# ejmahler/RustFFT

Measured on NVIDIA H100. Metric: batched complex-FFT GFLOP/s (5N log2 N), f32 forward, N=2^10..2^20, batch=4096/GPU, higher is better.
Workload: dtype f32

## Files before the change

rustfft_b200/csrc/common.h:

```cpp
#pragma once

#include <cstddef>
#include <cstdint>

#if defined(__CUDACC__)
#define B2_HD __host__ __device__ __forceinline__
#define B2_D __device__ __forceinline__
#else
#define B2_HD inline
#define B2_D inline
#endif

#if defined(__CUDA_ARCH__)
#define B2_UNROLL _Pragma("unroll")
#else
#define B2_UNROLL
#endif

#if !defined(B2_TW_ALL)
#if !defined(B2_TW_FEW)
#define B2_TW_FEW 1
#endif
#if !defined(B2_TWROW_FEW)
#define B2_TWROW_FEW 1
#endif
#endif

namespace b2 {

template <typename T>
struct alignas(2 * sizeof(T)) cx {
    T x, y;
};

template <typename T> B2_HD cx<T> mk(T x, T y) { cx<T> r; r.x = x; r.y = y; return r; }

template <typename T> B2_HD cx<T> operator+(cx<T> a, cx<T> b) { return mk<T>(a.x + b.x, a.y + b.y); }
template <typename T> B2_HD cx<T> operator-(cx<T> a, cx<T> b) { return mk<T>(a.x - b.x, a.y - b.y); }
template <typename T> B2_HD cx<T> cmul(cx<T> a, cx<T> w) {
#if defined(__CUDA_ARCH__)
    if constexpr (sizeof(T) == 4) return mk<T>(__fmaf_rn(-a.y, w.y, __fmul_rn(a.x, w.x)), __fmaf_rn(a.x, w.y, __fmul_rn(a.y, w.x)));
#endif
    return mk<T>(a.x * w.x - a.y * w.y, a.x * w.y + a.y * w.x);
}
template <typename T> B2_HD cx<T> cmulc(cx<T> a, cx<T> w) {
#if defined(__CUDA_ARCH__)
    if constexpr (sizeof(T) == 4) return mk<T>(__fmaf_rn(a.y, w.y, __fmul_rn(a.x, w.x)), __fmaf_rn(-a.x, w.y, __fmul_rn(a.y, w.x)));
#endif
    return mk<T>(a.x * w.x + a.y * w.y, a.y * w.x - a.x * w.y);
}
template <typename T> B2_HD cx<T> scale(cx<T> a, T s) { return mk<T>(a.x * s, a.y * s); }
template <typename T> B2_HD cx<T> axpy(cx<T> a, T s, cx<T> b) {
#if defined(__CUDA_ARCH__)
    if constexpr (sizeof(T) == 4) return mk<T>(__fmaf_rn(b.x, s, a.x), __fmaf_rn(b.y, s, a.y));
#endif
    return mk<T>(a.x + s * b.x, a.y + s * b.y);
}
template <typename T> B2_HD cx<T> conj(cx<T> a) { return mk<T>(a.x, -a.y); }
template <typename T> B2_HD cx<T> mul_mi(cx<T> a) { return mk<T>(a.y, -a.x); }
template <typename T> B2_HD cx<T> add_mi(cx<T> a, cx<T> b) { return mk<T>(a.x + b.y, a.y - b.x); }
template <typename T> B2_HD cx<T> sub_mi(cx<T> a, cx<T> b) { return mk<T>(a.x - b.y, a.y + b.x); }
template <typename T> B2_HD cx<T> swap_ri(cx<T> a) { return mk<T>(a.y, a.x); }

template <typename T> B2_HD cx<T> ldg(const cx<T>* p) {
#if defined(__CUDA_ARCH__)
    cx<T> r;
    if constexpr (sizeof(T) == 4) {
        asm("ld.global.nc.L1::evict_last.v2.f32 {%0, %1}, [%2];" : "=f"(r.x), "=f"(r.y) : "l"(p));
    } else {
        asm("ld.global.nc.L1::evict_last.v2.f64 {%0, %1}, [%2];" : "=d"(r.x), "=d"(r.y) : "l"(p));
    }
    return r;
#else
    return *p;
#endif
}
template <typename T> B2_HD cx<T> ldg_stream(const cx<T>* p) {
#if defined(__CUDA_ARCH__)
    cx<T> r;
    if constexpr (sizeof(T) == 4) {
        asm("ld.global.nc.L1::no_allocate.v2.f32 {%0, %1}, [%2];" : "=f"(r.x), "=f"(r.y) : "l"(p));
    } else {
        asm("ld.global.nc.L1::no_allocate.v2.f64 {%0, %1}, [%2];" : "=d"(r.x), "=d"(r.y) : "l"(p));
    }
    return r;
#else
    return *p;
#endif
}
B2_HD uint32_t ldg_u32(const uint32_t* p) {
#if defined(__CUDA_ARCH__)
    return __ldg(p);
#else
    return *p;
#endif
}

#if defined(__CUDACC__)
B2_D unsigned long long l2_evict_first() {
    unsigned long long p;
    asm("createpolicy.fractional.L2::evict_first.b64 %0, 1.0;" : "=l"(p));
    return p;
}
B2_D unsigned long long l2_evict_last() {
    unsigned long long p;
    asm("createpolicy.fractional.L2::evict_last.b64 %0, 1.0;" : "=l"(p));
    return p;
}
#endif
template <typename T> B2_HD cx<T> ld_stream(const cx<T>* p) {
#if defined(__CUDA_ARCH__)
    cx<T> r;
    if constexpr (sizeof(T) == 4) {
        asm volatile("ld.global.L1::no_allocate.L2::cache_hint.v2.f32 {%0, %1}, [%2], %3;"
                     : "=f"(r.x), "=f"(r.y) : "l"(p), "l"(l2_evict_first()));
    } else {
        asm volatile("ld.global.L1::no_allocate.L2::cache_hint.v2.f64 {%0, %1}, [%2], %3;"
                     : "=d"(r.x), "=d"(r.y) : "l"(p), "l"(l2_evict_first()));
    }
    return r;
#else
    return *p;
#endif
}
template <typename T> B2_HD void st_stream(cx<T>* p, cx<T> v) {
#if defined(__CUDA_ARCH__)
    if constexpr (sizeof(T) == 4) {
        asm volatile("st.global.L1::no_allocate.L2::cache_hint.v2.f32 [%0], {%1, %2}, %3;" ::"l"(p), "f"(v.x), "f"(v.y),
                     "l"(l2_evict_first()) : "memory");
    } else {
        asm volatile("st.global.L1::no_allocate.L2::cache_hint.v2.f64 [%0], {%1, %2}, %3;" ::"l"(p), "d"(v.x), "d"(v.y),
                     "l"(l2_evict_first()) : "memory");
    }
#else
    *p = v;
#endif
}
template <typename T> B2_HD cx<T> ld_cs(const cx<T>* p) {
#if defined(__CUDA_ARCH__)
    if constexpr (sizeof(T) == 4) {
        float2 v = __ldcs(reinterpret_cast<const float2*>(p));
        return mk<T>(v.x, v.y);
    } else {
        double2 v = __ldcs(reinterpret_cast<const double2*>(p));
        return mk<T>(v.x, v.y);
    }
#else
    return *p;
#endif
}
template <typename T> B2_HD void st_cs(cx<T>* p, cx<T> v) {
#if defined(__CUDA_ARCH__)
    if constexpr (sizeof(T) == 4) {
        __stcs(reinterpret_cast<float2*>(p), make_float2(v.x, v.y));
    } else {
        __stcs(reinterpret_cast<double2*>(p), make_double2(v.x, v.y));
    }
// ... 77 lines not shown
```

rustfft_b200/csrc/engine.h:

```cpp
#pragma once
#include "butterfly.h"
#include "common.h"

namespace b2 {

B2_HD constexpr int hibit(int r) {
    int h = 1;
    while (2 * h <= r) h *= 2;
    return h;
}

B2_HD constexpr int ilog2_c(int r) {
    int l = 0;
    while ((1 << (l + 1)) <= r) ++l;
    return l;
}

enum Map { JF = 0, FF = 1 };

template <typename T_, int L_, int E_, int F_, typename RL_, int PS_ = 4>
struct Geo {
    using T = T_;
    using RL = RL_;
    static constexpr int L = L_, E = E_, F = F_, PS = PS_;
    static constexpr int TP = L / E;
    static constexpr int NT = F * TP;
    static constexpr int NS = RL::N;
    static constexpr int LPAD = L + (PS ? (L >> PS) : 0);
    static constexpr int UNIT = 128 / (2 * (int)sizeof(T_));
    static constexpr int LPR = (LPAD + UNIT - 1) / UNIT * UNIT;
    static constexpr int LP = (F <= 1) ? LPAD : (F >= UNIT ? LPR + 1 : LPR + UNIT / F);
    static constexpr int SMEM_ELEMS = (NS > 1) ? F * LP : 0;
    static constexpr int TW_ELEMS = RL::tw_total();
    static constexpr bool POW2 = RL::all_pow2() && ((TP & (TP - 1)) == 0);
    static B2_HD int sidx(int f, int e) { return f * LP + e + (PS ? (e >> PS) : 0); }
    static_assert(RL::product() == L, "radices must multiply to L");
    static_assert(L % E == 0, "E must divide L");
};

template <class G, Map M>
B2_HD void tid_to_fj(int tid, int& f, int& j) {
    if (M == JF) {
        f = tid / G::TP;
        j = tid - f * G::TP;
    } else {
        j = tid / G::F;
        f = tid - j * G::F;
    }
}

template <class G, Map M0, Map M1>
struct Engine {
    using T = typename G::T;
    using RL = typename G::RL;
    static constexpr int E = G::E;

    template <int S>
    struct TwRegs {
        static constexpr int R = RL::get(S);
        static constexpr int Q = E / R;
        static constexpr int LG = ilog2_c(R);
        cx<T> w[Q][LG > 0 ? LG : 1];
    };
    template <int S>
    static B2_HD void load_tw(int j, const cx<T>* tw, TwRegs<S>& t) {
        constexpr int R = RL::get(S);
        constexpr int p = RL::product(S);
        constexpr int Q = E / R;
        B2_UNROLL
        for (int u = 0; u < Q; ++u) {
            const int i = j + u * G::TP;
            const int k = (p == 1) ? 0 : (i % p);
            const cx<T>* tp = tw + RL::tw_offset(S) + k;
            B2_UNROLL
            for (int l = 0; l < TwRegs<S>::LG; ++l) t.w[u][l] = ldg(tp + ((1 << l) - 1) * p);
        }
    }

    template <int S>
    static B2_HD void stage(int f, int j, cx<T> (&v)[E], cx<T>* smem, const cx<T>* tw, const TwRegs<S>* pre = nullptr) {
        constexpr int R = RL::get(S);
        constexpr int p = RL::product(S);
        constexpr int Q = E / R;
        constexpr bool last = (S == G::NS - 1);
        static_assert(E % R == 0, "every radix must divide E");
        cx<T> out[E];
        B2_UNROLL
        for (int u = 0; u < Q; ++u) {
            const int i = j + u * G::TP;
            const int k = (p == 1) ? 0 : (i % p);
            cx<T> a[R];
            B2_UNROLL
            for (int r = 0; r < R; ++r) a[r] = v[u + r * Q];
            if (S > 0) {
                const cx<T>* t = tw + RL::tw_offset(S) + k;
#if defined(B2_TW_FEW)
                if constexpr (R >= 8 && (R & (R - 1)) == 0 && sizeof(T) == 4) {
                    cx<T> w[R];
                    B2_UNROLL
                    for (int r = 1, l = 0; r < R; r <<= 1, ++l) w[r] = pre ? pre->w[u][l] : ldg(t + (r - 1) * p);
                    B2_UNROLL
                    for (int r = 3; r < R; ++r)
                        if (r & (r - 1)) {
                            const int hi = hibit(r);
                            w[r] = cmul(w[hi], w[r - hi]);
                        }
                    B2_UNROLL
                    for (int r = 1; r < R; ++r) a[r] = cmul(a[r], w[r]);
                } else
#endif
                {
                    B2_UNROLL
                    for (int r = 1; r < R; ++r) a[r] = cmul(a[r], ldg(t + (r - 1) * p));
                }
            }
            Bfly<R, T>::run(a);
            if (last) {
                B2_UNROLL
                for (int m = 0; m < R; ++m) out[u + m * Q] = a[m];
            } else {
                const int base = (i - k) * R + k;
                if constexpr (G::POW2) {
                    cx<T>* wp = smem + G::sidx(f, base);
                    B2_UNROLL
                    for (int m = 0; m < R; ++m) wp[m * p + (G::PS ? ((m * p) >> G::PS) : 0)] = a[m];
                } else {
                    B2_UNROLL
                    for (int m = 0; m < R; ++m) smem[G::sidx(f, base + m * p)] = a[m];
                }
            }
        }
        if (last) {
            B2_UNROLL
            for (int q = 0; q < E; ++q) v[q] = out[q];
        }
    }

    template <int S>
    static B2_HD void read(int f, int j, cx<T> (&v)[E], const cx<T>* smem) {
        if constexpr (G::POW2) {
            const cx<T>* rp = smem + G::sidx(f, j);
            B2_UNROLL
            for (int q = 0; q < E; ++q) v[q] = rp[G::TP * q + (G::PS ? ((G::TP * q) >> G::PS) : 0)];
        } else {
            B2_UNROLL
            for (int q = 0; q < E; ++q) v[q] = smem[G::sidx(f, j + G::TP * q)];
        }
    }

    static constexpr int NPHASE = 2 * G::NS - 1;

    template <int P>
    static B2_HD void owner(int tid, int& f, int& j) {
        if (P == 0)
            tid_to_fj<G, M0>(tid, f, j);
        else
            tid_to_fj<G, M1>(tid, f, j);
    }
    static B2_HD void out_owner(int tid, int& f, int& j) { owner<NPHASE - 1>(tid, f, j); }

    template <int P>
    static B2_HD void phase(int tid, cx<T> (&v)[E], cx<T>* smem, const cx<T>* tw) {
        int f, j;
        owner<P>(tid, f, j);
        if constexpr (P == 0) {
            stage<0>(f, j, v, smem, tw);
        } else if constexpr (P % 2 == 1) {
            read<(P + 1) / 2>(f, j, v, smem);
        } else {
            stage<P / 2>(f, j, v, smem, tw);
        }
    }
    static B2_HD void last_phase_pre(int tid, cx<T> (&v)[E], cx<T>* smem, const cx<T>* tw, const TwRegs<G::NS - 1>& pre) {
        int f, j;
        owner<NPHASE - 1>(tid, f, j);
        stage<G::NS - 1>(f, j, v, smem, tw, &pre);
    }
};

}
```

rustfft_b200/csrc/fused.h:

```cpp
#pragma once
#include "kernels.h"

namespace b2 {

template <class KA, class KB, int NG_, int NS_>
struct FusedKernel {
    using T = typename KA::T;
    static constexpr int NG = NG_;
    static constexpr int NSTAGE = NS_;
    static constexpr int NTG = KA::NT;
    static_assert(KA::NT == KB::NT, "both passes use the same consumer-group size");
    static_assert(KA::TILE_BYTES == KB::TILE_BYTES, "both passes move tiles of the same size");
    static_assert(NTG % 32 == 0 && NSTAGE <= 8 && NG <= 8, "geometry");
    static constexpr int NT = NG * NTG + 96;
    static constexpr int NQ = 2;
    static constexpr size_t STAGE_BYTES = ((KA::SMEM_BYTES > KB::SMEM_BYTES ? KA::SMEM_BYTES : KB::SMEM_BYTES) + 127) / 128 * 128;
    static constexpr size_t CTRL_BYTES = 512;
    static constexpr size_t SMEM_BYTES = (size_t)NSTAGE * STAGE_BYTES + CTRL_BYTES + 128;
    struct Params {
        typename KA::Params a;
        typename KB::Params b;
        FlowSched sched;
        uint32_t* ctl;
        unsigned long long* trace;
        uint32_t flags;
    };
};

static constexpr uint32_t FUSED_TRACE_CTAS = 16, FUSED_TRACE_WORDS = 4096;
inline uint64_t fused_trace_bytes() { return (uint64_t)FUSED_TRACE_CTAS * 4 * FUSED_TRACE_WORDS * 8; }

#if defined(__CUDACC__)
struct FusedTrace {
    unsigned long long* base;
    uint32_t n;
    B2_D void init(unsigned long long* trace, int role) {
        base = (trace != nullptr && blockIdx.x < FUSED_TRACE_CTAS) ? trace + ((size_t)blockIdx.x * 4 + role) * FUSED_TRACE_WORDS : nullptr;
        n = 0;
    }
    B2_D void stamp(uint32_t tag) {
        if (base != nullptr && n + 1 < FUSED_TRACE_WORDS) {
            unsigned long long t;
            asm volatile("mov.u64 %0, %%globaltimer;" : "=l"(t));
            base[n++] = (t << 8) | tag;
        }
    }
    B2_D void finish() {
        if (base != nullptr) base[FUSED_TRACE_WORDS - 1] = n;
    }
};
B2_D void red_release_add1(uint32_t* p) { asm volatile("red.release.gpu.global.add.u32 [%0], 1;" ::"l"(p) : "memory"); }
B2_D uint32_t ld_acquire_u32(const uint32_t* p) {
    uint32_t v;
    asm volatile("ld.acquire.gpu.global.u32 %0, [%1];" : "=r"(v) : "l"(p) : "memory");
    return v;
}
B2_D void fused_spin(uint32_t* ctl, const uint32_t* ctr, uint32_t target) {
    uint32_t spins = 0;
    while (ld_acquire_u32(ctr) < target) {
        __nanosleep(spins < 64 ? 20 : 200);
        if (++spins > (1u << 22) || (spins > 4096 && ld_relaxed_u32(ctl + 1) != 0)) {
            atomicExch(ctl + 1, 1u);
            break;
        }
    }
}

template <class KT, int P>
struct GroupPhases {
    static B2_D void run(const typename KT::Params& p, uint32_t bid, int ltid, typename KT::Regs& r, cx<typename KT::T>* buf, int bar_id,
                         uint64_t* release) {
        KT::template phase<P>(p, bid, ltid, r, buf);
        if constexpr (P + 2 < KT::NPHASE) {
            tma::named_bar_sync(bar_id, KT::NT);
            if constexpr (P + 3 == KT::NPHASE) {
                if (release != nullptr && ltid == 0) tma::mbar_arrive(release);
            }
            GroupPhases<KT, P + 1>::run(p, bid, ltid, r, buf, bar_id, release);
        }
    }
};

template <class KA, class KB, int NG, int NS>
__global__ void __launch_bounds__(FusedKernel<KA, KB, NG, NS>::NT, 1)
run_fused(const __grid_constant__ typename FusedKernel<KA, KB, NG, NS>::Params p) {
    using FK = FusedKernel<KA, KB, NG, NS>;
    using C = cx<typename FK::T>;
    constexpr int NTG = FK::NTG;
    extern __shared__ __align__(128) unsigned char smem_raw[];
    unsigned char* base = smem_raw + ((128u - (tma::smem_u32(smem_raw) & 127u)) & 127u);
    uint64_t* bars = reinterpret_cast<uint64_t*>(base + (size_t)NS * FK::STAGE_BYTES);
    uint64_t* full = bars;
    uint64_t* meta = bars + NS;
    uint64_t* outf = bars + 2 * NS;
    uint64_t* empty = bars + 3 * NS;
    uint64_t* q_full = bars + 4 * NS;
    uint64_t* q_empty = bars + 4 * NS + FK::NQ;
    volatile uint32_t* info = reinterpret_cast<volatile uint32_t*>(bars + 4 * NS + 2 * FK::NQ);
    volatile uint32_t* qent = info + 4 * NS;
    const int tid = (int)threadIdx.x;
    const int warp = tid >> 5, lane = tid & 31;
    const FlowSched& sc = p.sched;
    uint32_t* ready = p.ctl + FLOW_CTL_HEAD;
    uint32_t* freed = ready + sc.ring_w;
    if (tid == 0) {
        for (int s = 0; s < NS; ++s) {
            tma::mbar_init(&full[s], 1);
            tma::mbar_init(&meta[s], 1);
            tma::mbar_init(&outf[s], NTG / 32);
            tma::mbar_init(&empty[s], 1);
        }
        for (int q = 0; q < FK::NQ; ++q) {
            tma::mbar_init(&q_full[q], 1);
            tma::mbar_init(&q_empty[q], 1);
        }
        tma::fence_mbar_init();
    }
    __syncthreads();
    auto stage_buf = [&](uint32_t s) { return reinterpret_cast<C*>(base + (size_t)s * FK::STAGE_BYTES); };
    const uint32_t nq = (p.flags & 64u) ? (uint32_t)FK::NQ : 1u;

    if (warp == NG * NTG / 32 + 2) {
        if (lane == 0) {
            uint32_t k = 0;
            uint32_t ticket = atomicAdd(p.ctl, 1u);
            while (ticket < sc.total) {
                int kind;
                uint32_t t, tile;
                bool valid;
                sc.decode(ticket, kind, t, tile, valid);
                const uint32_t next = atomicAdd(p.ctl, 1u);
                if (valid) {
                    const FlowDep d = flow_dep(sc, p.ctl, ticket);
                    if (d.ptr != nullptr && ld_acquire_u32(d.ptr) < d.target) fused_spin(p.ctl, d.ptr, d.target);
                    if (d.ptr != nullptr) tma::fence_proxy_async_all();
                    const uint32_t q = k % nq, qph = (k / nq) & 1u;
                    tma::mbar_wait(&q_empty[q], qph ^ 1u);
                    qent[4 * q + 0] = (uint32_t)kind;
                    qent[4 * q + 1] = kind == 0 ? t * sc.TA + tile : t * sc.TB + tile;
                    qent[4 * q + 2] = t % sc.ring_w;
                    tma::mbar_arrive(&q_full[q]);
                    ++k;
                }
                ticket = next;
            }
            const uint32_t q = k % nq, qph = (k / nq) & 1u;
            tma::mbar_wait(&q_empty[q], qph ^ 1u);
            qent[4 * q + 0] = 2u;
            tma::mbar_arrive(&q_full[q]);
        }
    } else if (warp == NG * NTG / 32) {
        if (lane == 0) {
            uint32_t i = 0;
            FusedTrace tr;
            tr.init(p.trace, 0);
            const unsigned long long pol_a = (p.flags & 2u) ? l2_evict_first() : 0ull, pol_b = (p.flags & 4u) ? l2_evict_first() : 0ull;
            for (uint32_t k = 0;; ++k) {
                const uint32_t q = k % nq, qph = (k / nq) & 1u;
                tma::mbar_wait(&q_full[q], qph);
                const uint32_t kind = qent[4 * q + 0], bid = qent[4 * q + 1], slot = qent[4 * q + 2];
                tma::mbar_arrive(&q_empty[q]);
                if (kind == 2u) break;
                const uint32_t s = i % NS, ph = (i / NS) & 1u;
                tr.stamp(0x10u | kind);
                tma::mbar_wait(&empty[s], ph ^ 1u);
                tr.stamp(0x20u | s);
                info[4 * s + 0] = kind;
                info[4 * s + 1] = bid;
                info[4 * s + 2] = slot;
                tma::mbar_arrive(&meta[s]);
                if (kind == 0u)
                    KA::issue_load(p.a, bid, stage_buf(s), &full[s], pol_a);
                else
                    KB::issue_load(p.b, bid, stage_buf(s), &full[s], pol_b);
                tr.stamp(0x30u | s);
                ++i;
            }
            for (int g = 0; g < NG; ++g, ++i) {
                const uint32_t s = i % NS, ph = (i / NS) & 1u;
                tma::mbar_wait(&empty[s], ph ^ 1u);
                info[4 * s + 0] = 2u;
                tma::mbar_arrive(&meta[s]);
            }
            tr.finish();
        }
    } else if (warp == NG * NTG / 32 + 1) {
        if (lane == 0) {
            uint32_t* pending = nullptr;
            const unsigned long long pol_a = (p.flags & 8u) ? l2_evict_last() : 0ull, pol_b = (p.flags & 16u) ? l2_evict_first() : 0ull;
            FusedTrace tr;
            tr.init(p.trace, 1);
            uint32_t sph = 0;
            uint32_t held = 0xffffffffu;
            int ends = 0;
            uint32_t idle = 0;
            while (ends < NG) {
                bool any = false;
                for (uint32_t s = 0; s < (uint32_t)NS; ++s) {
                    if (!tma::mbar_test(&outf[s], (sph >> s) & 1u)) continue;
                    sph ^= 1u << s;
                    any = true;
                    const uint32_t kind = info[4 * s + 0], bid = info[4 * s + 1], slot = info[4 * s + 2];
                    if (kind == 2u) {
                        ++ends;
                        continue;
                    }
                    tr.stamp(0x40u | s);
                    if (kind == 0u)
                        KA::issue_store(p.a, bid, stage_buf(s), pol_a);
                    else
                        KB::issue_store(p.b, bid, stage_buf(s), pol_b);
                    tma::bulk_commit();
                    if (pending != nullptr) {
                        tma::bulk_wait<1>();
                        tma::fence_proxy_async_all();
                        red_release_add1(pending);
                        pending = nullptr;
                    }
                    tr.stamp(0x50u | s);
                    if (p.flags & 128u) {
                        if (held != 0xffffffffu) {
                            tma::bulk_wait_read<1>();
                            tma::mbar_arrive(&empty[held]);
                            tr.stamp(0x60u | held);
                        }
                        held = s;
                    } else {
                        tma::bulk_wait_read<0>();
                        tma::mbar_arrive(&empty[s]);
                        tr.stamp(0x60u | s);
                    }
                    if (kind == 0u) pending = ready + slot;
                }
                if (!any) {
                    if (held != 0xffffffffu) {
                        tma::bulk_wait_read<0>();
                        tma::mbar_arrive(&empty[held]);
                        tr.stamp(0x60u | held);
                        held = 0xffffffffu;
                    }
                    if (pending != nullptr) {
                        tma::bulk_wait<0>();
                        tma::fence_proxy_async_all();
                        red_release_add1(pending);
                        pending = nullptr;
                    }
                    __nanosleep(idle < 8 ? 32 : 128);
                    ++idle;
                } else {
                    idle = 0;
                }
            }
            tma::bulk_wait<0>();
            if (pending != nullptr) {
                tma::fence_proxy_async_all();
                red_release_add1(pending);
            }
            tr.finish();
        }
    } else {
        const int g = warp / (NTG / 32);
        const int ltid = tid - g * NTG;
        const int bar_id = 1 + g;
        constexpr bool DA = KA::DIRECT_OUT;
        constexpr bool DB = KB::DIRECT_OUT;
        FusedTrace tr;
        tr.init(ltid == 0 ? p.trace : nullptr, 2 + (g & 1));
        for (uint32_t i = (uint32_t)g;; i += NG) {
            const uint32_t s = i % NS, ph = (i / NS) & 1u;
            tma::mbar_wait(&meta[s], ph);
            tr.stamp(0x70u | s);
            const uint32_t kind = info[4 * s + 0], bid = info[4 * s + 1], slot = info[4 * s + 2];
            C* buf = stage_buf(s);
            bool via_smem = true;
            if (kind == 0u) {
                typename KA::Regs r;
                KA::prefetch(p.a, bid, ltid, r);
                tma::mbar_wait(&full[s], ph);
                tr.stamp(0x80u | s);
                if (!(p.flags & 1u)) {
                    GroupPhases<KA, 0>::run(p.a, bid, ltid, r, buf, bar_id, DA ? &empty[s] : nullptr);
                    if constexpr (DA) {
                        tma::named_bar_sync(bar_id, NTG);
                        if (ltid == 0) red_release_add1(ready + slot);
                        via_smem = false;
                    }
                } else if (DA) {
                    if (ltid == 0) {
                        tma::mbar_arrive(&empty[s]);
                        red_release_add1(ready + slot);
                    }
                    via_smem = false;
                } else {
                    tma::fence_proxy_async();
                }
            } else if (kind == 1u) {
                typename KB::Regs r;
                KB::prefetch(p.b, bid, ltid, r);
                tma::mbar_wait(&full[s], ph);
                tr.stamp(0x80u | s);
                if (!(p.flags & 1u)) {
                    GroupPhases<KB, 0>::run(p.b, bid, ltid, r, buf, bar_id, DB ? &empty[s] : nullptr);
                    if constexpr (DB) via_smem = false;
                } else if (DB) {
                    if (ltid == 0) tma::mbar_arrive(&empty[s]);
                    via_smem = false;
                } else {
                    tma::fence_proxy_async();
                }
            }
            if (via_smem) {
                __syncwarp();
                if (lane == 0) tma::mbar_arrive(&outf[s]);
            }
            tr.stamp(0x90u | s);
            if (kind == 1u && ltid == 0) red_release_add1(freed + slot);
            if (kind == 2u) break;
        }
        tr.finish();
    }
}
#endif

}
```

rustfft_b200/csrc/kernels.h:

```cpp
#pragma once
#include "engine.h"
#include "tma.h"

namespace b2 {

constexpr int default_min_blocks(int nt, int e = 16) {
    const int target_threads = e >= 24 ? 512 : 1024;
    const int b = target_threads / nt;
    return b < 1 ? 1 : (b > 8 ? 8 : b);
}

struct FastDiv {
    uint32_t d, mul, shift;
    B2_HD uint32_t div(uint32_t n) const {
        if (d == 1) return n;
#if defined(__CUDA_ARCH__)
        return __umulhi(n, mul) >> shift;
#else
        return (uint32_t)(((uint64_t)n * mul) >> 32) >> shift;
#endif
    }
};
inline FastDiv make_fastdiv(uint32_t d) {
    FastDiv f{d, 0, 0};
// ... 978 lines not shown
    static B2_HD void phase(const Params& p, uint32_t item, int tid, Regs& r, cx<T>* buf) {
        if constexpr (P == 0) {
            int f, j;
            tid_to_fj<G, JF>(tid, f, j);
            uint64_t g = (uint64_t)item * G::F + f;
            const auto st = p.xform.prep(g < p.n_fft ? g : p.n_fft - 1);
            const cx<T>* src = buf + f * G::L + j;
            B2_UNROLL
            for (int q = 0; q < G::E; ++q) r.v[q] = p.xform.apply(st, j + G::TP * q, src[G::TP * q]);
        } else {
            Eng::template phase<P - 1>(tid, r.v, buf, p.tw);
        }
        if constexpr (P == NPHASE - 1) {
            int f, j;
            Eng::out_owner(tid, f, j);
            const uint64_t g = (uint64_t)item * G::F + f;
            const auto st = p.store.prep(g, g < p.n_fft);
            B2_UNROLL
            for (int q = 0; q < G::E; ++q) p.store.put(st, j + G::TP * q, r.v[q]);
        }
    }
};

template <class G> struct RL_last_pow2 {
    static constexpr int R = G::RL::get(G::NS - 1);
    static constexpr bool value = R >= 8 && (R & (R - 1)) == 0;
};
template <class G, Map M0, Map M1, int ROLE, bool SW, int TILED = 0, bool DOUT = false>
struct TmaTileKernel {
    using T = typename G::T;
    using Eng = Engine<G, M0, M1>;
    static constexpr int NT = G::NT;
#if defined(B2_TMA_MINB)
    static constexpr int MIN_BLOCKS = (G::E >= 32 && sizeof(T) == 4) ? B2_TMA_MINB : default_min_blocks(G::NT, G::E);
#else
    static constexpr int MIN_BLOCKS = default_min_blocks(G::NT, G::E);
#endif
    static constexpr int NPHASE = Eng::NPHASE + 2;
    static constexpr size_t TILE_ELEMS = (size_t)G::F * G::L;
    static constexpr size_t BUF_ELEMS = ((TILE_ELEMS > (size_t)G::SMEM_ELEMS ? TILE_ELEMS : (size_t)G::SMEM_ELEMS) + 15) / 16 * 16;
    static constexpr size_t SMEM_BYTES = BUF_ELEMS * sizeof(cx<T>);
    static constexpr uint32_t TILE_BYTES = (uint32_t)(TILE_ELEMS * sizeof(cx<T>));
    static constexpr int BOX_ROWS = G::L < 256 ? G::L : 256;
    static constexpr int NBOX = G::L / BOX_ROWS;
    static_assert(G::NS >= 2, "single-stage sizes use the plain kernels");
    struct Params {
        TMap map_in;
        TMap map_out;
        const cx<T>* in;
        cx<T>* out;
        const cx<T>* tw;
        const cx<T>* full_tw;
        uint64_t n_fft;
        uint32_t lgN, lg_other;
        uint32_t z_in, z_out;
        uint32_t discard;
        const void* pf;
        uint32_t pf_bytes;
        const cx<T>* tw_lo;
        const cx<T>* tw_hi;
        uint32_t ring_w;
    };
    static constexpr bool DIRECT_OUT = (ROLE == 0 && TILED != 0) || (ROLE == 1 && DOUT);
    static constexpr int FO = (ROLE == 1 && TILED > 0) ? TILED : 1;
    static constexpr int TA = G::L / FO;
    static constexpr int TBOX = TA < 256 ? TA : 256;
    static constexpr bool TILED_IN = (ROLE == 1 && TILED > 0);
    static_assert(!TILED_IN || (G::L % FO == 0 && TA % TBOX == 0), "tile-major ring geometry");
    static B2_HD int tiled_base(int f, int j) {
        if constexpr (G::TP % FO == 0) return ((j / FO) * G::F + f) * FO + (j % FO);
        else return f * FO + j;
    }
    static constexpr int tiled_off(int q) {
        if (G::TP % FO == 0) return q * G::TP * G::F;
        return ((G::TP * q) / FO) * G::F * FO + (G::TP * q) % FO;
    }
    static_assert(!TILED_IN || G::TP % FO == 0 || FO % G::TP == 0, "powers of two");
    static B2_HD uint32_t zin(const Params& p, uint32_t b) { return (ROLE == 1 && p.ring_w) ? (p.z_in + b) % p.ring_w : p.z_in + b; }
    static B2_HD uint32_t zout(const Params& p, uint32_t b) { return (ROLE == 0 && p.ring_w) ? (p.z_out + b) % p.ring_w : p.z_out + b; }
    static constexpr bool PRE = (G::NS == 2) && sizeof(T) == 4 && ((RL_last_pow2<G>::value));
    static constexpr int LGE = ilog2_c(G::E);
    struct Regs {
        cx<T> v[G::E];
        typename Eng::template TwRegs<G::NS - 1> twl;
        cx<T> rw[LGE + 1];
    };
    struct Where { uint32_t b, c0; };
    static B2_HD void prefetch(const Params& p, uint32_t bid, int tid, Regs& r) {
        if constexpr (PRE) {
            int f, j;
            Eng::out_owner(tid, f, j);
            Eng::template load_tw<G::NS - 1>(j, p.tw, r.twl);
            if (ROLE == 1) {
                const Where w = where(p, bid);
                Eng::template owner<0>(tid, f, j);
                if (p.tw_lo != nullptr) {
                    const uint32_t k1 = w.c0 + (uint32_t)f, mask = (1u << p.lgN) - 1u;
                    auto tw2 = [&](uint32_t x) -> cx<T> {
                        const uint32_t m = (k1 * x) & mask;
                        return cmul(ldg(p.tw_hi + (m >> 10)), ldg(p.tw_lo + (m & 1023u)));
                    };
                    r.rw[0] = tw2((uint32_t)j);
                    B2_UNROLL
                    for (int l = 0; l < LGE; ++l) r.rw[l + 1] = tw2((uint32_t)(G::TP * (1 << l)));
                } else {
                    const cx<T>* t = p.full_tw + (uint64_t)(w.c0 + f) * G::L;
                    r.rw[0] = ldg_stream(t + j);
                    B2_UNROLL
                    for (int l = 0; l < LGE; ++l) r.rw[l + 1] = ldg_stream(t + G::TP * (1 << l));
                }
            }
        }
    }
    static B2_HD Where where(const Params& p, uint32_t bid) {
        const uint64_t g0 = (uint64_t)bid * G::F;
        return Where{(uint32_t)(g0 >> p.lg_other), (uint32_t)(g0 & ((1ull << p.lg_other) - 1))};
    }

#if defined(__CUDACC__)
    static B2_D void issue_load(const Params& p, uint32_t bid, cx<T>* buf, uint64_t* bar, unsigned long long pol = 0) {
        const Where w = where(p, bid);
        tma::mbar_arrive_expect_tx(bar, TILE_BYTES);
        if (ROLE == 0) {
            B2_UNROLL
            for (int k = 0; k < NBOX; ++k) {
                if (pol)
                    tma::tensor_g2s_3d_hint(buf + (size_t)k * BOX_ROWS * G::F, &p.map_in, (int)(2 * w.c0), k * BOX_ROWS, (int)zin(p, w.b), bar, pol);
                else
                    tma::tensor_g2s_3d(buf + (size_t)k * BOX_ROWS * G::F, &p.map_in, (int)(2 * w.c0), k * BOX_ROWS, (int)zin(p, w.b), bar);
            }
        } else if constexpr (TILED_IN) {
            B2_UNROLL
            for (int k = 0; k < TA / TBOX; ++k) {
                if (pol)
                    tma::tensor_g2s_4d_hint(buf + (size_t)k * TBOX * G::F * FO, &p.map_in, 0, (int)w.c0, k * TBOX, (int)zin(p, w.b), bar, pol);
                else
                    tma::tensor_g2s_4d(buf + (size_t)k * TBOX * G::F * FO, &p.map_in, 0, (int)w.c0, k * TBOX, (int)zin(p, w.b), bar);
            }
        } else {
            if (pol)
                tma::bulk_g2s_hint(buf, p.in + ((uint64_t)zin(p, w.b) << p.lgN) + (uint64_t)w.c0 * G::L, TILE_BYTES, bar, pol);
            else
                tma::bulk_g2s(buf, p.in + ((uint64_t)zin(p, w.b) << p.lgN) + (uint64_t)w.c0 * G::L, TILE_BYTES, bar);
            if (p.pf != nullptr && p.pf_bytes) tma::bulk_prefetch_l2(static_cast<const char*>(p.pf) + (uint64_t)bid * p.pf_bytes, p.pf_bytes);
        }
    }
    static B2_D void issue_store(const Params& p, uint32_t bid, const cx<T>* buf, unsigned long long pol = 0) {
        const Where w = where(p, bid);
        B2_UNROLL
        for (int k = 0; k < NBOX; ++k) {
            if (pol)
                tma::tensor_s2g_3d_hint(&p.map_out, (int)(2 * w.c0), k * BOX_ROWS, (int)zout(p, w.b), buf + (size_t)k * BOX_ROWS * G::F, pol);
            else
                tma::tensor_s2g_3d(&p.map_out, (int)(2 * w.c0), k * BOX_ROWS, (int)zout(p, w.b), buf + (size_t)k * BOX_ROWS * G::F);
        }
    }
#endif

    template <int P>
    static B2_HD void phase(const Params& p, uint32_t bid, int tid, Regs& r, cx<T>* buf) {
        if constexpr (P == 0) {
            const Where w = where(p, bid);
#if !defined(__CUDA_ARCH__)
            prefetch(p, bid, tid, r);
            if (tid == 0) {
                if (ROLE == 0) {
                    const cx<T>* src = p.in + ((uint64_t)zin(p, w.b) << p.lgN) + w.c0;
                    for (int e = 0; e < G::L; ++e)
                        for (int f = 0; f < G::F; ++f) buf[e * G::F + f] = src[((uint64_t)e << p.lg_other) + f];
                } else if constexpr (TILED_IN) {
                    const cx<T>* src = p.in + ((uint64_t)zin(p, w.b) << p.lgN);
                    for (int t = 0; t < TA; ++t)
                        for (int f = 0; f < G::F; ++f)
                            for (int c = 0; c < FO; ++c) buf[((size_t)t * G::F + f) * FO + c] = src[(size_t)t * TILE_ELEMS + (size_t)(w.c0 + f) * FO + c];
                } else {
                    const cx<T>* src = p.in + ((uint64_t)zin(p, w.b) << p.lgN) + (uint64_t)w.c0 * G::L;
                    for (size_t i = 0; i < TILE_ELEMS; ++i) buf[i] = src[i];
                }
            }
#endif
            int f, j;
            Eng::template owner<0>(tid, f, j);
            if (ROLE == 0) {
                const cx<T>* src = buf + (size_t)j * G::F + f;
                B2_UNROLL
                for (int q = 0; q < G::E; ++q) {
                    const cx<T> v = src[(size_t)G::TP * q * G::F];
                    r.v[q] = SW ? swap_ri(v) : v;
                }
            } else {
                const cx<T>* src = TILED_IN ? buf + tiled_base(f, j) : buf + (size_t)f * G::L + j;
                auto at = [&](int q) -> cx<T> { return TILED_IN ? src[tiled_off(q)] : src[G::TP * q]; };
                const cx<T>* t = p.full_tw + (uint64_t)(w.c0 + f) * G::L + j;
#if defined(B2_TWROW_FEW)
                if constexpr (sizeof(T) == 4) {
                    cx<T> wq[G::E];
                    const cx<T> a = PRE ? r.rw[0] : ldg_stream(t);
                    B2_UNROLL
                    for (int q = 1, l = 1; q < G::E; q <<= 1, ++l) wq[q] = PRE ? r.rw[l] : ldg_stream(t - j + G::TP * q);
                    B2_UNROLL
                    for (int q = 3; q < G::E; ++q)
                        if (q & (q - 1)) wq[q] = cmul(wq[hibit(q)], wq[q - hibit(q)]);
                    r.v[0] = cmul(at(0), a);
                    B2_UNROLL
                    for (int q = 1; q < G::E; ++q) r.v[q] = cmul(at(q), cmul(a, wq[q]));
                } else
#endif
                {
                    B2_UNROLL
                    for (int q = 0; q < G::E; ++q) r.v[q] = cmul(at(q), ldg_stream(t + G::TP * q));
                }
            }
        } else if constexpr (P < NPHASE - 1) {
            if constexpr (P == 1 && ROLE == 1) {
                if (p.discard) {
                    const Where w = where(p, bid);
                    if constexpr (TILED_IN) {
                        constexpr uint32_t CHUNK = (uint32_t)(G::F * FO * sizeof(cx<T>));
                        if constexpr (CHUNK % 128 == 0) {
                            constexpr uint32_t LPC = CHUNK / 128;
                            const char* base = reinterpret_cast<const char*>(p.in + ((uint64_t)zin(p, w.b) << p.lgN) + (uint64_t)w.c0 * FO);
                            for (uint32_t l = (uint32_t)tid; l < TILE_BYTES / 128; l += (uint32_t)G::NT)
                                l2_discard_line(base + (size_t)(l / LPC) * TILE_BYTES + (size_t)(l % LPC) * 128);
                        }
                    } else {
                        const char* base = reinterpret_cast<const char*>(p.in + ((uint64_t)zin(p, w.b) << p.lgN) + (uint64_t)w.c0 * G::L);
                        for (uint32_t l = (uint32_t)tid; l < TILE_BYTES / 128; l += (uint32_t)G::NT) l2_discard_line(base + (size_t)l * 128);
                    }
                }
            }
            if constexpr (P == NPHASE - 2 && PRE)
                Eng::last_phase_pre(tid, r.v, buf, p.tw, r.twl);
            else
                Eng::template phase<P - 1>(tid, r.v, buf, p.tw);
            if constexpr (P == NPHASE - 2) {
                int f, j;
                Eng::out_owner(tid, f, j);
                if constexpr (ROLE == 1 && DOUT) {
                    const Where w = where(p, bid);
                    cx<T>* dst = p.out + ((uint64_t)zout(p, w.b) << p.lgN) + w.c0 + f + ((size_t)j << p.lg_other);
                    B2_UNROLL
                    for (int q = 0; q < G::E; ++q) st_cs(dst + ((size_t)(G::TP * q) << p.lg_other), SW ? swap_ri(r.v[q]) : r.v[q]);
                } else if constexpr (DIRECT_OUT) {
                    const Where w = where(p, bid);
                    cx<T>* dst = p.out + ((uint64_t)zout(p, w.b) << p.lgN) + (size_t)(w.c0 / G::F) * TILE_ELEMS + (size_t)j * G::F + f;
                    B2_UNROLL
                    for (int q = 0; q < G::E; ++q) dst[(size_t)G::TP * q * G::F] = r.v[q];
                } else {
                    cx<T>* dst = buf + (size_t)j * G::F + f;
                    B2_UNROLL
                    for (int q = 0; q < G::E; ++q) dst[(size_t)G::TP * q * G::F] = (ROLE == 1 && SW) ? swap_ri(r.v[q]) : r.v[q];
#if defined(__CUDA_ARCH__)
                    tma::fence_proxy_async();
#endif
                }
            }
        } else {
            if (tid == 0 && !DIRECT_OUT) {
                const Where w = where(p, bid);
#if defined(__CUDA_ARCH__)
                issue_store(p, bid, buf);
                tma::bulk_commit();
                tma::bulk_wait_read0();
#else
                cx<T>* dst = p.out + ((uint64_t)zout(p, w.b) << p.lgN) + w.c0;
                for (int e = 0; e < G::L; ++e)
                    for (int f = 0; f < G::F; ++f) dst[((uint64_t)e << p.lg_other) + f] = buf[e * G::F + f];
#endif
            }
        }
    }
};

struct FlowSched {
    uint32_t batch, TA, TB, D, ring_w, per_round, m, a_big, n_rounds, total;
    B2_HD void decode(uint32_t ticket, int& kind, uint32_t& t, uint32_t& tile, bool& valid) const {
        const uint32_t r = ticket / per_round, i = ticket - r * per_round;
        const uint32_t period = m + 1, k = i / period, j = i - k * period;
        const bool big = j < m;
        tile = big ? k * m + j : k;
        if (big == (a_big != 0)) {
            kind = 0;
            t = r;
            valid = r < batch;
        } else {
            kind = 1;
            t = r - D;
            valid = r >= D && t < batch;
        }
    }
};
inline bool make_flow_sched(FlowSched& s, uint64_t batch, uint32_t TA, uint32_t TB, uint32_t W) {
    s.TA = TA;
    s.TB = TB;
    s.ring_w = W;
    uint32_t D = W > 2 ? W / 2 : 1;
    if ((uint64_t)D > batch) D = (uint32_t)batch;
    if (D < 1) D = 1;
    s.D = D;
    s.per_round = TA + TB;
    s.a_big = TA >= TB ? 1u : 0u;
    s.m = s.a_big ? TA / TB : TB / TA;
    const uint64_t rounds = batch + D, total = rounds * s.per_round;
    if (batch >= (1ull << 31) || total >= (1ull << 31)) return false;
    s.batch = (uint32_t)batch;
    s.n_rounds = (uint32_t)rounds;
    s.total = (uint32_t)total;
    return true;
}
static constexpr uint32_t FLOW_CTL_HEAD = 32;
inline uint64_t flow_ctl_bytes(uint32_t W) { return ((uint64_t)(FLOW_CTL_HEAD + 2 * W) * 4 + 255) / 256 * 256; }

template <class KA, class KB>
struct FlowKernel {
    using T = typename KA::T;
    static constexpr int NT = KA::NT > KB::NT ? KA::NT : KB::NT;
    static constexpr int MIN_BLOCKS = KA::MIN_BLOCKS < KB::MIN_BLOCKS ? KA::MIN_BLOCKS : KB::MIN_BLOCKS;
// ... 295 lines not shown
```

rustfft_b200/csrc/tma.h:

```cpp
#pragma once
#include <cstdint>

#include "common.h"

#if defined(__CUDACC__)
namespace b2 {
namespace tma {

B2_D uint32_t smem_u32(const void* p) { return (uint32_t)__cvta_generic_to_shared(p); }

B2_D void mbar_init(uint64_t* bar, uint32_t count) {
    asm volatile("mbarrier.init.shared::cta.b64 [%0], %1;" ::"r"(smem_u32(bar)), "r"(count) : "memory");
}
B2_D void fence_mbar_init() { asm volatile("fence.mbarrier_init.release.cluster;" ::: "memory"); }
B2_D void fence_proxy_async() { asm volatile("fence.proxy.async.shared::cta;" ::: "memory"); }

B2_D void mbar_arrive_expect_tx(uint64_t* bar, uint32_t bytes) {
    asm volatile("mbarrier.arrive.expect_tx.shared::cta.b64 _, [%0], %1;" ::"r"(smem_u32(bar)), "r"(bytes) : "memory");
}
B2_D void mbar_wait(uint64_t* bar, uint32_t parity) {
    asm volatile(
        "{\n"
        ".reg .pred p;\n"
        "WAIT_%=:\n"
// ... 3 lines not shown
        "DONE_%=:\n"
        "}\n" ::"r"(smem_u32(bar)),
        "r"(parity)
        : "memory");
}
B2_D void bulk_g2s(void* smem_dst, const void* gmem_src, uint32_t bytes, uint64_t* bar) {
    asm volatile("cp.async.bulk.shared::cluster.global.mbarrier::complete_tx::bytes [%0], [%1], %2, [%3];" ::"r"(
                     smem_u32(smem_dst)),
                 "l"(gmem_src), "r"(bytes), "r"(smem_u32(bar))
                 : "memory");
}
B2_D void bulk_s2g(void* gmem_dst, const void* smem_src, uint32_t bytes) {
    asm volatile("cp.async.bulk.global.shared::cta.bulk_group [%0], [%1], %2;" ::"l"(gmem_dst), "r"(smem_u32(smem_src)),
                 "r"(bytes)
                 : "memory");
}
B2_D void tensor_g2s_3d(void* smem_dst, const void* tmap, int x, int y, int z, uint64_t* bar) {
    asm volatile("cp.async.bulk.tensor.3d.shared::cluster.global.mbarrier::complete_tx::bytes [%0], [%1, {%3, %4, %5}], [%2];" ::"r"(
                     smem_u32(smem_dst)),
                 "l"(tmap), "r"(smem_u32(bar)), "r"(x), "r"(y), "r"(z)
                 : "memory");
}
B2_D void tensor_g2s_4d(void* smem_dst, const void* tmap, int x, int y, int z, int w, uint64_t* bar) {
    asm volatile("cp.async.bulk.tensor.4d.shared::cluster.global.mbarrier::complete_tx::bytes [%0], [%1, {%3, %4, %5, %6}], [%2];" ::"r"(
                     smem_u32(smem_dst)),
                 "l"(tmap), "r"(smem_u32(bar)), "r"(x), "r"(y), "r"(z), "r"(w)
                 : "memory");
}
B2_D void tensor_g2s_4d_hint(void* smem_dst, const void* tmap, int x, int y, int z, int w, uint64_t* bar, unsigned long long pol) {
    asm volatile(
        "cp.async.bulk.tensor.4d.shared::cluster.global.mbarrier::complete_tx::bytes.L2::cache_hint [%0], [%1, {%3, %4, %5, %6}], [%2], %7;" ::"r"(
            smem_u32(smem_dst)),
        "l"(tmap), "r"(smem_u32(bar)), "r"(x), "r"(y), "r"(z), "r"(w), "l"(pol)
        : "memory");
}
B2_D void tensor_s2g_3d(const void* tmap, int x, int y, int z, const void* smem_src) {
    asm volatile("cp.async.bulk.tensor.3d.global.shared::cta.bulk_group [%0, {%2, %3, %4}], [%1];" ::"l"(tmap),
                 "r"(smem_u32(smem_src)), "r"(x), "r"(y), "r"(z)
                 : "memory");
}
B2_D void tensor_g2s_3d_hint(void* smem_dst, const void* tmap, int x, int y, int z, uint64_t* bar, unsigned long long pol) {
    asm volatile(
        "cp.async.bulk.tensor.3d.shared::cluster.global.mbarrier::complete_tx::bytes.L2::cache_hint [%0], [%1, {%3, %4, %5}], [%2], %6;" ::"r"(
            smem_u32(smem_dst)),
        "l"(tmap), "r"(smem_u32(bar)), "r"(x), "r"(y), "r"(z), "l"(pol)
        : "memory");
}
B2_D void tensor_s2g_3d_hint(const void* tmap, int x, int y, int z, const void* smem_src, unsigned long long pol) {
    asm volatile("cp.async.bulk.tensor.3d.global.shared::cta.bulk_group.L2::cache_hint [%0, {%2, %3, %4}], [%1], %5;" ::"l"(tmap),
                 "r"(smem_u32(smem_src)), "r"(x), "r"(y), "r"(z), "l"(pol)
                 : "memory");
}
B2_D void bulk_g2s_hint(void* smem_dst, const void* gmem_src, uint32_t bytes, uint64_t* bar, unsigned long long pol) {
    asm volatile("cp.async.bulk.shared::cluster.global.mbarrier::complete_tx::bytes.L2::cache_hint [%0], [%1], %2, [%3], %4;" ::"r"(
                     smem_u32(smem_dst)),
                 "l"(gmem_src), "r"(bytes), "r"(smem_u32(bar)), "l"(pol)
                 : "memory");
}
B2_D void bulk_prefetch_l2(const void* gmem_src, uint32_t bytes) {
    asm volatile("cp.async.bulk.prefetch.L2.global [%0], %1;" ::"l"(gmem_src), "r"(bytes) : "memory");
}
B2_D void mbar_arrive(uint64_t* bar) {
    asm volatile("mbarrier.arrive.shared::cta.b64 _, [%0];" ::"r"(smem_u32(bar)) : "memory");
}
B2_D bool mbar_test(uint64_t* bar, uint32_t parity) {
    uint32_t ok;
    asm volatile(
        "{\n"
        ".reg .pred p;\n"
        "mbarrier.test_wait.parity.shared::cta.b64 p, [%1], %2;\n"
        "selp.u32 %0, 1, 0, p;\n"
        "}\n"
        : "=r"(ok)
        : "r"(smem_u32(bar)), "r"(parity)
        : "memory");
    return ok != 0;
}
B2_D void fence_proxy_async_all() { asm volatile("fence.proxy.async;" ::: "memory"); }
template <int N> B2_D void bulk_wait() { asm volatile("cp.async.bulk.wait_group %0;" ::"n"(N) : "memory"); }
template <int N> B2_D void bulk_wait_read() { asm volatile("cp.async.bulk.wait_group.read %0;" ::"n"(N) : "memory"); }
B2_D void named_bar_sync(int id, int count) { asm volatile("bar.sync %0, %1;" ::"r"(id), "r"(count) : "memory"); }
B2_D void bulk_commit() { asm volatile("cp.async.bulk.commit_group;" ::: "memory"); }
B2_D void bulk_wait_read0() { asm volatile("cp.async.bulk.wait_group.read 0;" ::: "memory"); }

}
}
#endif
```

Measured before the change: 8783.

## Rebalance registers with setmaxnreg and replace twiddle preload registers with L1 prefetch

The fused kernel's service warps grow from 96 to 128 threads so they form a whole warpgroup. That warpgroup lowers its register cap with setmaxnreg, and the consumer warps raise theirs to a computed budget. The last-stage twiddle preload, which held twiddles in registers, becomes an L1 prefetch, cutting register pressure. The twiddle-product computation is also interleaved into the multiply loop. The aim is to avoid spills in the consumer warps. The cost is an extra 32 idle threads and twiddle loads that may now miss L1.

```diff
diff --git a/rustfft_b200/csrc/common.h b/rustfft_b200/csrc/common.h
--- a/rustfft_b200/csrc/common.h
+++ b/rustfft_b200/csrc/common.h
@@ -73,6 +73,13 @@
     return r;
 #else
     return *p;
+#endif
+}
+template <typename T> B2_HD void prefetch_l1(const T* p) {
+#if defined(__CUDA_ARCH__)
+    asm volatile("prefetch.global.L1 [%0];" ::"l"(p));
+#else
+    (void)p;
 #endif
 }
 template <typename T> B2_HD cx<T> ldg_stream(const cx<T>* p) {
diff --git a/rustfft_b200/csrc/engine.h b/rustfft_b200/csrc/engine.h
--- a/rustfft_b200/csrc/engine.h
+++ b/rustfft_b200/csrc/engine.h
@@ -56,14 +56,7 @@
     static constexpr int E = G::E;
 
     template <int S>
-    struct TwRegs {
-        static constexpr int R = RL::get(S);
-        static constexpr int Q = E / R;
-        static constexpr int LG = ilog2_c(R);
-        cx<T> w[Q][LG > 0 ? LG : 1];
-    };
-    template <int S>
-    static B2_HD void load_tw(int j, const cx<T>* tw, TwRegs<S>& t) {
+    static B2_HD void prefetch_tw(int j, const cx<T>* tw) {
         constexpr int R = RL::get(S);
         constexpr int p = RL::product(S);
         constexpr int Q = E / R;
@@ -73,12 +66,12 @@
             const int k = (p == 1) ? 0 : (i % p);
             const cx<T>* tp = tw + RL::tw_offset(S) + k;
             B2_UNROLL
-            for (int l = 0; l < TwRegs<S>::LG; ++l) t.w[u][l] = ldg(tp + ((1 << l) - 1) * p);
+            for (int r = 1; r < R; r <<= 1) prefetch_l1(tp + (r - 1) * p);
         }
     }
 
     template <int S>
-    static B2_HD void stage(int f, int j, cx<T> (&v)[E], cx<T>* smem, const cx<T>* tw, const TwRegs<S>* pre = nullptr) {
+    static B2_HD void stage(int f, int j, cx<T> (&v)[E], cx<T>* smem, const cx<T>* tw) {
         constexpr int R = RL::get(S);
         constexpr int p = RL::product(S);
         constexpr int Q = E / R;
@@ -98,7 +91,7 @@
                 if constexpr (R >= 8 && (R & (R - 1)) == 0 && sizeof(T) == 4) {
                     cx<T> w[R];
                     B2_UNROLL
-                    for (int r = 1, l = 0; r < R; r <<= 1, ++l) w[r] = pre ? pre->w[u][l] : ldg(t + (r - 1) * p);
+                    for (int r = 1; r < R; r <<= 1) w[r] = ldg(t + (r - 1) * p);
                     B2_UNROLL
                     for (int r = 3; r < R; ++r)
                         if (r & (r - 1)) {
@@ -171,11 +164,6 @@
             stage<P / 2>(f, j, v, smem, tw);
         }
     }
-    static B2_HD void last_phase_pre(int tid, cx<T> (&v)[E], cx<T>* smem, const cx<T>* tw, const TwRegs<G::NS - 1>& pre) {
-        int f, j;
-        owner<NPHASE - 1>(tid, f, j);
-        stage<G::NS - 1>(f, j, v, smem, tw, &pre);
-    }
 };
 
 }
diff --git a/rustfft_b200/csrc/fused.h b/rustfft_b200/csrc/fused.h
--- a/rustfft_b200/csrc/fused.h
+++ b/rustfft_b200/csrc/fused.h
@@ -12,7 +12,14 @@
     static_assert(KA::NT == KB::NT, "both passes use the same consumer-group size");
     static_assert(KA::TILE_BYTES == KB::TILE_BYTES, "both passes move tiles of the same size");
     static_assert(NTG % 32 == 0 && NSTAGE <= 8 && NG <= 8, "geometry");
-    static constexpr int NT = NG * NTG + 96;
+    static_assert(NG * NTG % 128 == 0, "consumer groups fill whole warpgroups");
+    static constexpr int NT = NG * NTG + 128;
+    static constexpr int SVC_WARP = NG * NTG / 32;
+    static constexpr int LAUNCH_REGS = 65536 / NT / 8 * 8;
+    static constexpr int SVC_REGS = 32;
+    static constexpr int CONS_REGS = (LAUNCH_REGS * NT - SVC_REGS * 128) / (NG * NTG) / 8 * 8;
+    static_assert(CONS_REGS * NG * NTG + SVC_REGS * 128 <= LAUNCH_REGS * NT && CONS_REGS >= LAUNCH_REGS && CONS_REGS <= 256,
+                  "setmaxnreg budgets must not overcommit the registers the launch granted");
     static constexpr int NQ = 2;
     static constexpr size_t STAGE_BYTES = ((KA::SMEM_BYTES > KB::SMEM_BYTES ? KA::SMEM_BYTES : KB::SMEM_BYTES) + 127) / 128 * 128;
     static constexpr size_t CTRL_BYTES = 512;
@@ -120,145 +127,149 @@
     auto stage_buf = [&](uint32_t s) { return reinterpret_cast<C*>(base + (size_t)s * FK::STAGE_BYTES); };
     const uint32_t nq = (p.flags & 64u) ? (uint32_t)FK::NQ : 1u;
 
-    if (warp == NG * NTG / 32 + 2) {
-        if (lane == 0) {
-            uint32_t k = 0;
-            uint32_t ticket = atomicAdd(p.ctl, 1u);
-            while (ticket < sc.total) {
-                int kind;
-                uint32_t t, tile;
-                bool valid;
-                sc.decode(ticket, kind, t, tile, valid);
-                const uint32_t next = atomicAdd(p.ctl, 1u);
-                if (valid) {
-                    const FlowDep d = flow_dep(sc, p.ctl, ticket);
-                    if (d.ptr != nullptr && ld_acquire_u32(d.ptr) < d.target) fused_spin(p.ctl, d.ptr, d.target);
-                    if (d.ptr != nullptr) tma::fence_proxy_async_all();
+    if (warp >= FK::SVC_WARP) {
+        tma::setmaxnreg_dec<FK::SVC_REGS>();
+        if (warp == FK::SVC_WARP + 2) {
+            if (lane == 0) {
+                uint32_t k = 0;
+                uint32_t ticket = atomicAdd(p.ctl, 1u);
+                while (ticket < sc.total) {
+                    int kind;
+                    uint32_t t, tile;
+                    bool valid;
+                    sc.decode(ticket, kind, t, tile, valid);
+                    const uint32_t next = atomicAdd(p.ctl, 1u);
+                    if (valid) {
+                        const FlowDep d = flow_dep(sc, p.ctl, ticket);
+                        if (d.ptr != nullptr && ld_acquire_u32(d.ptr) < d.target) fused_spin(p.ctl, d.ptr, d.target);
+                        if (d.ptr != nullptr) tma::fence_proxy_async_all();
+                        const uint32_t q = k % nq, qph = (k / nq) & 1u;
+                        tma::mbar_wait(&q_empty[q], qph ^ 1u);
+                        qent[4 * q + 0] = (uint32_t)kind;
+                        qent[4 * q + 1] = kind == 0 ? t * sc.TA + tile : t * sc.TB + tile;
+                        qent[4 * q + 2] = t % sc.ring_w;
+                        tma::mbar_arrive(&q_full[q]);
+                        ++k;
+                    }
+                    ticket = next;
+                }
+                const uint32_t q = k % nq, qph = (k / nq) & 1u;
+                tma::mbar_wait(&q_empty[q], qph ^ 1u);
+                qent[4 * q + 0] = 2u;
+                tma::mbar_arrive(&q_full[q]);
+            }
+        } else if (warp == FK::SVC_WARP) {
+            if (lane == 0) {
+                uint32_t i = 0;
+                FusedTrace tr;
+                tr.init(p.trace, 0);
+                const unsigned long long pol_a = (p.flags & 2u) ? l2_evict_first() : 0ull, pol_b = (p.flags & 4u) ? l2_evict_first() : 0ull;
+                for (uint32_t k = 0;; ++k) {
                     const uint32_t q = k % nq, qph = (k / nq) & 1u;
-                    tma::mbar_wait(&q_empty[q], qph ^ 1u);
-                    qent[4 * q + 0] = (uint32_t)kind;
-                    qent[4 * q + 1] = kind == 0 ? t * sc.TA + tile : t * sc.TB + tile;
-                    qent[4 * q + 2] = t % sc.ring_w;
-                    tma::mbar_arrive(&q_full[q]);
-                    ++k;
-                }
-                ticket = next;
-            }
-            const uint32_t q = k % nq, qph = (k / nq) & 1u;
-            tma::mbar_wait(&q_empty[q], qph ^ 1u);
-            qent[4 * q + 0] = 2u;
-            tma::mbar_arrive(&q_full[q]);
-        }
-    } else if (warp == NG * NTG / 32) {
-        if (lane == 0) {
-            uint32_t i = 0;
-            FusedTrace tr;
-            tr.init(p.trace, 0);
-            const unsigned long long pol_a = (p.flags & 2u) ? l2_evict_first() : 0ull, pol_b = (p.flags & 4u) ? l2_evict_first() : 0ull;
-            for (uint32_t k = 0;; ++k) {
-                const uint32_t q = k % nq, qph = (k / nq) & 1u;
-                tma::mbar_wait(&q_full[q], qph);
-                const uint32_t kind = qent[4 * q + 0], bid = qent[4 * q + 1], slot = qent[4 * q + 2];
-                tma::mbar_arrive(&q_empty[q]);
-                if (kind == 2u) break;
-                const uint32_t s = i % NS, ph = (i / NS) & 1u;
-                tr.stamp(0x10u | kind);
-                tma::mbar_wait(&empty[s], ph ^ 1u);
-                tr.stamp(0x20u | s);
-                info[4 * s + 0] = kind;
-                info[4 * s + 1] = bid;
-                info[4 * s + 2] = slot;
-                tma::mbar_arrive(&meta[s]);
-                if (kind == 0u)
-                    KA::issue_load(p.a, bid, stage_buf(s), &full[s], pol_a);
-                else
-                    KB::issue_load(p.b, bid, stage_buf(s), &full[s], pol_b);
-                tr.stamp(0x30u | s);
-                ++i;
-            }
-            for (int g = 0; g < NG; ++g, ++i) {
-                const uint32_t s = i % NS, ph = (i / NS) & 1u;
-                tma::mbar_wait(&empty[s], ph ^ 1u);
-                info[4 * s + 0] = 2u;
-                tma::mbar_arrive(&meta[s]);
-            }
-            tr.finish();
-        }
-    } else if (warp == NG * NTG / 32 + 1) {
-        if (lane == 0) {
-            uint32_t* pending = nullptr;
-            const unsigned long long pol_a = (p.flags & 8u) ? l2_evict_last() : 0ull, pol_b = (p.flags & 16u) ? l2_evict_first() : 0ull;
-            FusedTrace tr;
-            tr.init(p.trace, 1);
-            uint32_t sph = 0;
-            uint32_t held = 0xffffffffu;
-            int ends = 0;
-            uint32_t idle = 0;
-            while (ends < NG) {
-                bool any = false;
-                for (uint32_t s = 0; s < (uint32_t)NS; ++s) {
-                    if (!tma::mbar_test(&outf[s], (sph >> s) & 1u)) continue;
-                    sph ^= 1u << s;
-                    any = true;
-                    const uint32_t kind = info[4 * s + 0], bid = info[4 * s + 1], slot = info[4 * s + 2];
-                    if (kind == 2u) {
-                        ++ends;
-                        continue;
-                    }
-                    tr.stamp(0x40u | s);
+                    tma::mbar_wait(&q_full[q], qph);
+                    const uint32_t kind = qent[4 * q + 0], bid = qent[4 * q + 1], slot = qent[4 * q + 2];
+                    tma::mbar_arrive(&q_empty[q]);
+                    if (kind == 2u) break;
+                    const uint32_t s = i % NS, ph = (i / NS) & 1u;
+                    tr.stamp(0x10u | kind);
+                    tma::mbar_wait(&empty[s], ph ^ 1u);
+                    tr.stamp(0x20u | s);
+                    info[4 * s + 0] = kind;
+                    info[4 * s + 1] = bid;
+                    info[4 * s + 2] = slot;
+                    tma::mbar_arrive(&meta[s]);
                     if (kind == 0u)
-                        KA::issue_store(p.a, bid, stage_buf(s), pol_a);
+                        KA::issue_load(p.a, bid, stage_buf(s), &full[s], pol_a);
                     else
-                        KB::issue_store(p.b, bid, stage_buf(s), pol_b);
-                    tma::bulk_commit();
-                    if (pending != nullptr) {
-                        tma::bulk_wait<1>();
-                        tma::fence_proxy_async_all();
-                        red_release_add1(pending);
-                        pending = nullptr;
-                    }
-                    tr.stamp(0x50u | s);
-                    if (p.flags & 128u) {
+                        KB::issue_load(p.b, bid, stage_buf(s), &full[s], pol_b);
+                    tr.stamp(0x30u | s);
+                    ++i;
+                }
+                for (int g = 0; g < NG; ++g, ++i) {
+                    const uint32_t s = i % NS, ph = (i / NS) & 1u;
+                    tma::mbar_wait(&empty[s], ph ^ 1u);
+                    info[4 * s + 0] = 2u;
+                    tma::mbar_arrive(&meta[s]);
+                }
+                tr.finish();
+            }
+        } else if (warp == FK::SVC_WARP + 1) {
+            if (lane == 0) {
+                uint32_t* pending = nullptr;
+                const unsigned long long pol_a = (p.flags & 8u) ? l2_evict_last() : 0ull, pol_b = (p.flags & 16u) ? l2_evict_first() : 0ull;
+                FusedTrace tr;
+                tr.init(p.trace, 1);
+                uint32_t sph = 0;
+                uint32_t held = 0xffffffffu;
+                int ends = 0;
+                uint32_t idle = 0;
+                while (ends < NG) {
+                    bool any = false;
+                    for (uint32_t s = 0; s < (uint32_t)NS; ++s) {
+                        if (!tma::mbar_test(&outf[s], (sph >> s) & 1u)) continue;
+                        sph ^= 1u << s;
+                        any = true;
+                        const uint32_t kind = info[4 * s + 0], bid = info[4 * s + 1], slot = info[4 * s + 2];
+                        if (kind == 2u) {
+                            ++ends;
+                            continue;
+                        }
+                        tr.stamp(0x40u | s);
+                        if (kind == 0u)
+                            KA::issue_store(p.a, bid, stage_buf(s), pol_a);
+                        else
+                            KB::issue_store(p.b, bid, stage_buf(s), pol_b);
+                        tma::bulk_commit();
+                        if (pending != nullptr) {
+                            tma::bulk_wait<1>();
+                            tma::fence_proxy_async_all();
+                            red_release_add1(pending);
+                            pending = nullptr;
+                        }
+                        tr.stamp(0x50u | s);
+                        if (p.flags & 128u) {
+                            if (held != 0xffffffffu) {
+                                tma::bulk_wait_read<1>();
+                                tma::mbar_arrive(&empty[held]);
+                                tr.stamp(0x60u | held);
+                            }
+                            held = s;
+                        } else {
+                            tma::bulk_wait_read<0>();
+                            tma::mbar_arrive(&empty[s]);
+                            tr.stamp(0x60u | s);
+                        }
+                        if (kind == 0u) pending = ready + slot;
+                    }
+                    if (!any) {
                         if (held != 0xffffffffu) {
-                            tma::bulk_wait_read<1>();
+                            tma::bulk_wait_read<0>();
                             tma::mbar_arrive(&empty[held]);
                             tr.stamp(0x60u | held);
-                        }
-                        held = s;
+                            held = 0xffffffffu;
+                        }
+                        if (pending != nullptr) {
+                            tma::bulk_wait<0>();
+                            tma::fence_proxy_async_all();
+                            red_release_add1(pending);
+                            pending = nullptr;
+                        }
+                        __nanosleep(idle < 8 ? 32 : 128);
+                        ++idle;
                     } else {
-                        tma::bulk_wait_read<0>();
-                        tma::mbar_arrive(&empty[s]);
-                        tr.stamp(0x60u | s);
-                    }
-                    if (kind == 0u) pending = ready + slot;
-                }
-                if (!any) {
-                    if (held != 0xffffffffu) {
-                        tma::bulk_wait_read<0>();
-                        tma::mbar_arrive(&empty[held]);
-                        tr.stamp(0x60u | held);
-                        held = 0xffffffffu;
-                    }
-                    if (pending != nullptr) {
-                        tma::bulk_wait<0>();
-                        tma::fence_proxy_async_all();
-                        red_release_add1(pending);
-                        pending = nullptr;
-                    }
-                    __nanosleep(idle < 8 ? 32 : 128);
-                    ++idle;
-                } else {
-                    idle = 0;
-                }
-            }
-            tma::bulk_wait<0>();
-            if (pending != nullptr) {
-                tma::fence_proxy_async_all();
-                red_release_add1(pending);
-            }
-            tr.finish();
+                        idle = 0;
+                    }
+                }
+                tma::bulk_wait<0>();
+                if (pending != nullptr) {
+                    tma::fence_proxy_async_all();
+                    red_release_add1(pending);
+                }
+                tr.finish();
+            }
         }
     } else {
+        tma::setmaxnreg_inc<FK::CONS_REGS>();
         const int g = warp / (NTG / 32);
         const int ltid = tid - g * NTG;
         const int bar_id = 1 + g;
diff --git a/rustfft_b200/csrc/kernels.h b/rustfft_b200/csrc/kernels.h
--- a/rustfft_b200/csrc/kernels.h
+++ b/rustfft_b200/csrc/kernels.h
@@ -1084,7 +1084,6 @@
     static constexpr int LGE = ilog2_c(G::E);
     struct Regs {
         cx<T> v[G::E];
-        typename Eng::template TwRegs<G::NS - 1> twl;
         cx<T> rw[LGE + 1];
     };
     struct Where { uint32_t b, c0; };
@@ -1092,7 +1091,7 @@
         if constexpr (PRE) {
             int f, j;
             Eng::out_owner(tid, f, j);
-            Eng::template load_tw<G::NS - 1>(j, p.tw, r.twl);
+            Eng::template prefetch_tw<G::NS - 1>(j, p.tw);
             if (ROLE == 1) {
                 const Where w = where(p, bid);
                 Eng::template owner<0>(tid, f, j);
@@ -1200,12 +1199,12 @@
                     const cx<T> a = PRE ? r.rw[0] : ldg_stream(t);
                     B2_UNROLL
                     for (int q = 1, l = 1; q < G::E; q <<= 1, ++l) wq[q] = PRE ? r.rw[l] : ldg_stream(t - j + G::TP * q);
-                    B2_UNROLL
-                    for (int q = 3; q < G::E; ++q)
-                        if (q & (q - 1)) wq[q] = cmul(wq[hibit(q)], wq[q - hibit(q)]);
                     r.v[0] = cmul(at(0), a);
                     B2_UNROLL
-                    for (int q = 1; q < G::E; ++q) r.v[q] = cmul(at(q), cmul(a, wq[q]));
+                    for (int q = 1; q < G::E; ++q) {
+                        if (q & (q - 1)) wq[q] = cmul(wq[hibit(q)], wq[q - hibit(q)]);
+                        r.v[q] = cmul(at(q), cmul(a, wq[q]));
+                    }
                 } else
 #endif
                 {
@@ -1231,10 +1230,7 @@
                     }
                 }
             }
-            if constexpr (P == NPHASE - 2 && PRE)
-                Eng::last_phase_pre(tid, r.v, buf, p.tw, r.twl);
-            else
-                Eng::template phase<P - 1>(tid, r.v, buf, p.tw);
+            Eng::template phase<P - 1>(tid, r.v, buf, p.tw);
             if constexpr (P == NPHASE - 2) {
                 int f, j;
                 Eng::out_owner(tid, f, j);
diff --git a/rustfft_b200/csrc/tma.h b/rustfft_b200/csrc/tma.h
--- a/rustfft_b200/csrc/tma.h
+++ b/rustfft_b200/csrc/tma.h
@@ -109,6 +109,8 @@
 B2_D void named_bar_sync(int id, int count) { asm volatile("bar.sync %0, %1;" ::"r"(id), "r"(count) : "memory"); }
 B2_D void bulk_commit() { asm volatile("cp.async.bulk.commit_group;" ::: "memory"); }
 B2_D void bulk_wait_read0() { asm volatile("cp.async.bulk.wait_group.read 0;" ::: "memory"); }
+template <int REGS> B2_D void setmaxnreg_dec() { asm volatile("setmaxnreg.dec.sync.aligned.u32 %0;" ::"n"(REGS)); }
+template <int REGS> B2_D void setmaxnreg_inc() { asm volatile("setmaxnreg.inc.sync.aligned.u32 %0;" ::"n"(REGS)); }
 
 }
 }
```

New measurement: 10280, median of 6. +17.0%, better.
